# ErlerPhilipp/points2surf

Hardware: NVIDIA H100
Metric: SDF queries/sec at grid_res=256 (higher is better)
Workload: dtype f16 operands / f32 accumulate (wgmma); hi/lo split f16 (fp32-level) for FC tails and guard-band recompute

## Files before the change

points2surf_b200/csrc/net_tc.cu:

```cuda
#include "model.cuh"
#include "tc_ptx.cuh"

namespace p2s {

using namespace ptx;

namespace {

constexpr int kTile = 64;
constexpr int kWG = 2;
constexpr int kThreads = 128 * kWG;
constexpr uint32_t kAct2Bytes = kTile * 128 * 2;
template <bool PRECISE>
struct Cfg {
    static constexpr int kChunks = PRECISE ? 1 : 4;
    static constexpr int kSplit = 8 / kChunks;
    static constexpr uint32_t kChunkBytes = PRECISE ? 65536u : 32768u;
    static constexpr uint32_t kW3Bytes = kChunks * kChunkBytes;
    static constexpr uint32_t kMidScale = PRECISE ? 2u : 1u;
    static constexpr uint32_t kMidBytes = (8192u + 8192u + 16384u) * kMidScale;
    static constexpr uint32_t kPerqBytes = PRECISE ? 16384u : 8192u;
    static constexpr uint32_t kOffMid = kW3Bytes;
    static constexpr uint32_t kWgPerq = kAct2Bytes * kMidScale;
    static constexpr uint32_t kWgWq = kWgPerq + kPerqBytes;
    static constexpr uint32_t kWgBytes = kWgWq + 192 * 4;
    static constexpr uint32_t kOffWg = kOffMid + kMidBytes;
    static constexpr uint32_t kOffBias = kOffWg + kWG * kWgBytes;
    static constexpr uint32_t kSmemBytes = kOffBias + 320 * 4;
};
static_assert(Cfg<false>::kSmemBytes <= 232448 && Cfg<true>::kSmemBytes <= 232448, "shared memory budget");

struct Seg {
    const float* ptr;
    int n;
    int tiles;
    int center;
};

struct PassParams {
    Seg seg[2];
    const float* query;
    const float* R;
    int tiles_per_query;
    int B;
    const float* W0;
    const float* b0;
    int num_mid;
    int mid_N[3];
    const uint8_t* mid_img[3];
    const float* mid_bias[3];
    int perq_layer;
    const uint8_t* perq_img;
    const uint8_t* w3_img;
    float* out;
};

__device__ __forceinline__ uint32_t pack_relu(float a, float b) {
    uint32_t r;
    asm("cvt.rn.relu.satfinite.f16x2.f32 %0, %1, %2;" : "=r"(r) : "f"(b), "f"(a));
    return r;
}
__device__ __forceinline__ void pack_relu_split(float a, float b, uint32_t& hi, uint32_t& lo) {
    hi = pack_relu(a, b);
    const float2 hf = __half22float2(*reinterpret_cast<const __half2*>(&hi));
    lo = pack_half2(fmaxf(a, 0.f) - hf.x, fmaxf(b, 0.f) - hf.y);
}
template <bool PRECISE>
__device__ __forceinline__ void pack_act(float a, float b, uint32_t& hi, uint32_t& lo) {
    if (PRECISE) pack_relu_split(a, b, hi, lo);
    else hi = pack_relu(a, b);
}

template <bool PRECISE, int R>
__device__ __forceinline__ void mid_mma(float (&d)[R], const uint32_t (&a)[4], const uint32_t (&al)[4], uint64_t w, uint64_t w_lo, uint32_t acc) {
    if (R == 32) {
        auto& d32 = reinterpret_cast<float (&)[32]>(d);
        if (PRECISE) { wgmma_rs_n64(d32, al, w, acc); wgmma_rs_n64(d32, a, w_lo, 1); wgmma_rs_n64(d32, a, w, 1); }
        else wgmma_rs_n64(d32, a, w, acc);
    } else {
        auto& d64 = reinterpret_cast<float (&)[64]>(d);
        if (PRECISE) { wgmma_rs_n128(d64, al, w, acc); wgmma_rs_n128(d64, a, w_lo, 1); wgmma_rs_n128(d64, a, w, 1); }
        else wgmma_rs_n128(d64, a, w, acc);
    }
}

template <bool PRECISE>
__global__ void __launch_bounds__(kThreads, 1) pointnet_pass_kernel(const PassParams p) {
    using C = Cfg<PRECISE>;
    constexpr int kL = PRECISE ? 4 : 1;
    extern __shared__ __align__(1024) uint8_t smem[];
    float* s_bias = reinterpret_cast<float*>(smem + C::kOffBias);
    const int tid = threadIdx.x, wg = tid >> 7, t = tid & 127, lane = tid & 31, q4 = lane & 3;
    const int r0 = (t >> 5) * 16 + (lane >> 2);
    const int part = blockIdx.x % C::kSplit;
    const int stream = blockIdx.x / C::kSplit, nstreams = gridDim.x / C::kSplit;
    const int nq = (p.B > stream) ? (p.B - stream + nstreams - 1) / nstreams : 0;
    const int tpq = p.tiles_per_query;
    uint32_t mid_off[3] = {0, 0, 0};
    {
        uint32_t o = 0;
        for (int l = 0; l < p.num_mid; ++l) { mid_off[l] = o; o += (uint32_t)p.mid_N[l] * 128u * C::kMidScale; }
    }

    if (nq > 0) {
        const uint4* src = reinterpret_cast<const uint4*>(p.w3_img + (size_t)part * C::kW3Bytes);
        uint4* dst = reinterpret_cast<uint4*>(smem);
        for (uint32_t i = tid; i < C::kW3Bytes / 16; i += kThreads) dst[i] = src[i];
        for (int l = 0; l < p.num_mid; ++l) {
            if (l == p.perq_layer) continue;
            const uint4* s = reinterpret_cast<const uint4*>(p.mid_img[l]);
            uint4* d = reinterpret_cast<uint4*>(smem + C::kOffMid + mid_off[l]);
            for (uint32_t i = tid; i < (uint32_t)p.mid_N[l] * 8u * C::kMidScale; i += kThreads) d[i] = s[i];
        }
    }
    {
        int off = 0;
        for (int l = 0; l < p.num_mid; ++l) {
            for (int i = tid; i < p.mid_N[l]; i += kThreads) s_bias[off + i] = p.mid_bias[l][i];
            off += p.mid_N[l];
        }
        for (int i = tid; i < 64; i += kThreads) s_bias[256 + i] = p.b0[i];
    }
    fence_proxy_async_smem();
    __syncthreads();

    uint8_t* wsm = smem + C::kOffWg + wg * C::kWgBytes;
    uint8_t* act2 = wsm;
    uint8_t* perq = wsm + C::kWgPerq;
    float* wq = reinterpret_cast<float*>(wsm + C::kWgWq);
    const float* s_b0 = s_bias + 256;
    const uint32_t bar_id = 1 + (uint32_t)wg;
    auto wg_sync = [&]() { asm volatile("bar.sync %0, 128;" ::"r"(bar_id) : "memory"); };
    const uint64_t dsc_act2 = make_smem_desc(smem_u32(act2), 128, 2048);
    const uint64_t dsc_w3 = make_smem_desc(smem_u32(smem), 128, 2048);
    uint64_t dsc_mid[3], dsc_mid_lo[3];
    for (int l = 0; l < 3; ++l) {
        const bool pq = l == p.perq_layer;
        dsc_mid[l] = make_smem_desc(pq ? smem_u32(perq) : smem_u32(smem + C::kOffMid) + mid_off[l], 128, 1024);
        dsc_mid_lo[l] = dsc_mid[l] + (uint64_t)((pq ? 8192u : (uint32_t)p.mid_N[l] * 128u) >> 4);
    }

    for (int qi = wg; qi < nq; qi += kWG) {
        const size_t q = (size_t)stream + (size_t)qi * nstreams;
        wg_sync();
        if (t < 64) {
            const float w0 = p.W0[t * 3 + 0], w1 = p.W0[t * 3 + 1], w2 = p.W0[t * 3 + 2];
            float r[9] = {1.f, 0.f, 0.f, 0.f, 1.f, 0.f, 0.f, 0.f, 1.f};
            if (p.R) {
#pragma unroll
                for (int i = 0; i < 9; ++i) r[i] = p.R[q * 9 + i];
            }
            wq[0 * 64 + t] = w0 * r[0] + w1 * r[3] + w2 * r[6];
            wq[1 * 64 + t] = w0 * r[1] + w1 * r[4] + w2 * r[7];
            wq[2 * 64 + t] = w0 * r[2] + w1 * r[5] + w2 * r[8];
        }
        if (p.perq_layer >= 0) {
            const uint4* s = reinterpret_cast<const uint4*>(p.perq_img + q * C::kPerqBytes);
            uint4* d = reinterpret_cast<uint4*>(perq);
            for (uint32_t i = t; i < C::kPerqBytes / 16; i += 128) d[i] = s[i];
            fence_proxy_async_smem();
        }
        wg_sync();
        float rmax[4 * C::kChunks];
#pragma unroll
        for (int i = 0; i < 4 * C::kChunks; ++i) rmax[i] = -INFINITY;
        for (int tq = 0; tq < tpq; ++tq) {
            const int sgi = tq < p.seg[0].tiles ? 0 : 1;
            const Seg& sg = p.seg[sgi];
            float cx = 0.f, cy = 0.f, cz = 0.f;
            if (sg.center) { cx = p.query[q * 3 + 0]; cy = p.query[q * 3 + 1]; cz = p.query[q * 3 + 2]; }
            float px[2], py[2], pz[2];
#pragma unroll
            for (int h = 0; h < 2; ++h) {
                int local = (tq - (sgi ? p.seg[0].tiles : 0)) * kTile + r0 + 8 * h;
                if (local >= sg.n) local = 0;
                const float* src = sg.ptr + (q * sg.n + local) * 3;
                px[h] = src[0] - cx; py[h] = src[1] - cy; pz[h] = src[2] - cz;
            }
            uint32_t a[4][4], al[4][kL];
#pragma unroll
            for (int kk = 0; kk < 4; ++kk) {
#pragma unroll
                for (int hc = 0; hc < 2; ++hc) {
                    const int ch = kk * 16 + hc * 8 + 2 * q4;
                    const float2 wx = *reinterpret_cast<const float2*>(wq + 0 * 64 + ch);
                    const float2 wy = *reinterpret_cast<const float2*>(wq + 1 * 64 + ch);
                    const float2 wz = *reinterpret_cast<const float2*>(wq + 2 * 64 + ch);
                    const float2 bb = *reinterpret_cast<const float2*>(s_b0 + ch);
#pragma unroll
                    for (int h = 0; h < 2; ++h) {
                        const float v0 = fmaf(wx.x, px[h], fmaf(wy.x, py[h], fmaf(wz.x, pz[h], bb.x)));
                        const float v1 = fmaf(wx.y, px[h], fmaf(wy.y, py[h], fmaf(wz.y, pz[h], bb.y)));
                        pack_act<PRECISE>(v0, v1, a[kk][hc * 2 + h], al[kk][PRECISE ? hc * 2 + h : 0]);
                    }
                }
            }
            int boff = 0;
            for (int l = 0; l < p.num_mid; ++l) {
                const float* bl = s_bias + boff;
                const uint64_t w = dsc_mid[l], w_lo = dsc_mid_lo[l];
                if (l < p.num_mid - 1) {
                    float d[32];
#pragma unroll
                    for (int i = 0; i < 32; ++i) d[i] = 0.f;
                    wgmma_fence();
#pragma unroll
                    for (int ks = 0; ks < 4; ++ks)
                        mid_mma<PRECISE>(d, a[ks], reinterpret_cast<const uint32_t (&)[4]>(al[PRECISE ? ks : 0]), w + (uint64_t)(ks * 16), w_lo + (uint64_t)(ks * 16), ks > 0);
                    wgmma_commit();
                    wgmma_wait<0>();
                    fence_regs(d);
#pragma unroll
                    for (int j = 0; j < 8; ++j) {
                        const float2 bb = *reinterpret_cast<const float2*>(bl + 8 * j + 2 * q4);
                        pack_act<PRECISE>(d[4 * j] + bb.x, d[4 * j + 1] + bb.y, a[j >> 1][(j & 1) * 2], al[j >> 1][PRECISE ? (j & 1) * 2 : 0]);
                        pack_act<PRECISE>(d[4 * j + 2] + bb.x, d[4 * j + 3] + bb.y, a[j >> 1][(j & 1) * 2 + 1], al[j >> 1][PRECISE ? (j & 1) * 2 + 1 : 0]);
                    }
                } else {
                    float d[64];
#pragma unroll
                    for (int i = 0; i < 64; ++i) d[i] = 0.f;
                    wgmma_fence();
#pragma unroll
                    for (int ks = 0; ks < 4; ++ks)
                        mid_mma<PRECISE>(d, a[ks], reinterpret_cast<const uint32_t (&)[4]>(al[PRECISE ? ks : 0]), w + (uint64_t)(ks * 16), w_lo + (uint64_t)(ks * 16), ks > 0);
                    wgmma_commit();
                    wgmma_wait<0>();
                    fence_regs(d);
                    wg_sync();
#pragma unroll
                    for (int j = 0; j < 16; ++j) {
                        const int k = 8 * j + 2 * q4;
                        const float2 bb = *reinterpret_cast<const float2*>(bl + k);
#pragma unroll
                        for (int h = 0; h < 2; ++h) {
                            const int pt = r0 + 8 * h;
                            const uint32_t off = (uint32_t)(pt >> 3) * 2048u + (uint32_t)j * 128u + (uint32_t)(pt & 7) * 16u + (uint32_t)q4 * 4u;
                            uint32_t hi, lo = 0;
                            pack_act<PRECISE>(d[4 * j + 2 * h] + bb.x, d[4 * j + 2 * h + 1] + bb.y, hi, lo);
                            *reinterpret_cast<uint32_t*>(act2 + off) = hi;
                            if (PRECISE) *reinterpret_cast<uint32_t*>(act2 + kAct2Bytes + off) = lo;
                        }
                    }
                    fence_proxy_async_smem();
                    wg_sync();
                }
                boff += p.mid_N[l];
            }
#pragma unroll
            for (int c = 0; c < C::kChunks; ++c) {
                float d0[32], d1[32];
#pragma unroll
                for (int i = 0; i < 32; ++i) { d0[i] = 0.f; d1[i] = 0.f; }
                const uint64_t wa = dsc_w3 + (uint64_t)((uint32_t)c * (C::kChunkBytes >> 4)), wb = wa + (uint64_t)(16384u >> 4);
                wgmma_fence();
#pragma unroll
                for (int ks = 0; ks < 8; ++ks) {
                    const uint64_t x = dsc_act2 + (uint64_t)(ks * 16), o = (uint64_t)(ks * 16);
                    if (PRECISE) {
                        const uint64_t x_lo = x + (uint64_t)(kAct2Bytes >> 4), lo = (uint64_t)(32768u >> 4);
                        wgmma_ss_n64(d0, wa + lo + o, x, ks > 0); wgmma_ss_n64(d0, wa + o, x_lo, 1); wgmma_ss_n64(d0, wa + o, x, 1);
                        wgmma_ss_n64(d1, wb + lo + o, x, ks > 0); wgmma_ss_n64(d1, wb + o, x_lo, 1); wgmma_ss_n64(d1, wb + o, x, 1);
                    } else {
                        wgmma_ss_n64(d0, wa + o, x, ks > 0);
                        wgmma_ss_n64(d1, wb + o, x, ks > 0);
                    }
                }
                wgmma_commit();
                wgmma_wait<0>();
                fence_regs(d0);
                fence_regs(d1);
#pragma unroll
                for (int j = 0; j < 8; ++j) {
                    rmax[4 * c + 0] = fmaxf(rmax[4 * c + 0], fmaxf(d0[4 * j], d0[4 * j + 1]));
                    rmax[4 * c + 1] = fmaxf(rmax[4 * c + 1], fmaxf(d0[4 * j + 2], d0[4 * j + 3]));
                    rmax[4 * c + 2] = fmaxf(rmax[4 * c + 2], fmaxf(d1[4 * j], d1[4 * j + 1]));
                    rmax[4 * c + 3] = fmaxf(rmax[4 * c + 3], fmaxf(d1[4 * j + 2], d1[4 * j + 3]));
                }
            }
        }
#pragma unroll
        for (int i = 0; i < 4 * C::kChunks; ++i) {
            rmax[i] = fmaxf(rmax[i], __shfl_xor_sync(0xffffffffu, rmax[i], 1));
            rmax[i] = fmaxf(rmax[i], __shfl_xor_sync(0xffffffffu, rmax[i], 2));
        }
        if (q4 == 0) {
#pragma unroll
            for (int i = 0; i < 4 * C::kChunks; ++i)
                p.out[q * 1024 + (size_t)((part * C::kChunks + (i >> 2)) * 128 + ((i >> 1) & 1) * 64 + r0 + (i & 1) * 8)] = rmax[i];
        }
    }
}

__global__ void pack_kmajor_kernel(const float* __restrict__ W, int rows, int K, int row0, uint32_t sbo, uint8_t* __restrict__ img, int lo) {
    int e = blockIdx.x * blockDim.x + threadIdx.x;
    if (e >= rows * K) return;
    int r = e / K, k = e % K;
    uint32_t off = (uint32_t)(r >> 3) * sbo + (uint32_t)(k >> 3) * 128u + (uint32_t)(r & 7) * 16u + (uint32_t)(k & 7) * 2u;
    const float w = W[(size_t)(row0 + r) * K + k];
    const __half h = __float2half_rn(w);
    *reinterpret_cast<__half*>(img + off) = lo ? __float2half_rn(w - __half2float(h)) : h;
}

__global__ void pack_perq_kernel(const float* __restrict__ W, int64_t B, uint8_t* __restrict__ img) {
    int64_t e = (int64_t)blockIdx.x * blockDim.x + threadIdx.x;
    if (e >= B * 4096) return;
    int64_t b = e >> 12;
    int r = (int)((e >> 6) & 63), k = (int)(e & 63);
    uint32_t off = (uint32_t)(r >> 3) * 1024u + (uint32_t)(k >> 3) * 128u + (uint32_t)(r & 7) * 16u + (uint32_t)(k & 7) * 2u;
    *reinterpret_cast<__half*>(img + b * 8192 + off) = __float2half_rn(W[e]);
}

__global__ void __launch_bounds__(256) fold_w1_kernel(const float* __restrict__ W1, const float* __restrict__ T, int64_t B, uint8_t* __restrict__ img) {
    __shared__ float sW[64][65];
    __shared__ __align__(16) float sT[64][68];
    const int64_t b = blockIdx.x;
    const int tid = threadIdx.x;
    for (int e = tid; e < 4096; e += 256) {
        const int r = e >> 6, c = e & 63;
        sW[r][c] = W1[e];
        sT[r][c] = T[b * 4096 + e] + (r == c ? 1.0f : 0.0f);
    }
    __syncthreads();
    const int o = tid >> 2, i0 = (tid & 3) * 16;
    float acc[16];
#pragma unroll
    for (int i = 0; i < 16; ++i) acc[i] = 0.f;
    for (int j = 0; j < 64; ++j) {
        const float w = sW[o][j];
#pragma unroll
        for (int i4 = 0; i4 < 4; ++i4) {
            const float4 t4 = *reinterpret_cast<const float4*>(&sT[j][i0 + 4 * i4]);
            acc[4 * i4 + 0] = fmaf(w, t4.x, acc[4 * i4 + 0]);
            acc[4 * i4 + 1] = fmaf(w, t4.y, acc[4 * i4 + 1]);
            acc[4 * i4 + 2] = fmaf(w, t4.z, acc[4 * i4 + 2]);
            acc[4 * i4 + 3] = fmaf(w, t4.w, acc[4 * i4 + 3]);
        }
    }
    uint8_t* dst = img + b * 8192 + (uint32_t)(o >> 3) * 1024u + (uint32_t)(o & 7) * 16u;
#pragma unroll
    for (int h = 0; h < 2; ++h) {
        uint32_t v[4];
#pragma unroll
        for (int e = 0; e < 4; ++e) v[e] = pack_half2(acc[h * 8 + 2 * e], acc[h * 8 + 2 * e + 1]);
        *reinterpret_cast<uint4*>(dst + (uint32_t)(i0 / 8 + h) * 128u) = make_uint4(v[0], v[1], v[2], v[3]);
    }
}

__global__ void fold_fc3_kernel(const float* __restrict__ W1, const float* __restrict__ Wfc3, const float* __restrict__ bfc3,
                                float* __restrict__ G, float* __restrict__ g0) {
    const int oi = blockIdx.x;
    const int o = oi >> 6, i = oi & 63;
    const int k = threadIdx.x;
    float acc = 0.f;
    for (int j = 0; j < 64; ++j) acc = fmaf(W1[o * 64 + j], Wfc3[(size_t)(j * 64 + i) * 256 + k], acc);
    G[(size_t)oi * 256 + k] = acc;
    if (k == 0) {
        float b = W1[o * 64 + i];
        for (int j = 0; j < 64; ++j) b = fmaf(W1[o * 64 + j], bfc3[j * 64 + i], b);
        g0[oi] = b;
    }
}

__global__ void transpose64_kernel(const float* __restrict__ in, float* __restrict__ out, int64_t B) {
    int64_t e = (int64_t)blockIdx.x * blockDim.x + threadIdx.x;
    if (e >= B * 4096) return;
    int64_t b = e >> 12;
    int i = (int)((e >> 6) & 63), j = (int)(e & 63);
    out[e] = in[b * 4096 + j * 64 + i];
}

__global__ void guard_flag_kernel(const float* __restrict__ logits, int64_t B, float band, int32_t* __restrict__ list, int* __restrict__ count, int64_t base, int64_t cap) {
    int64_t i = (int64_t)blockIdx.x * blockDim.x + threadIdx.x;
    if (i >= B) return;
    if (fabsf(logits[i * 2 + 1]) < band) {
        int slot = atomicAdd(count, 1);
        if (slot < cap) list[slot] = (int32_t)(base + i);
    }
}
__global__ void guard_gather_kernel(const float* __restrict__ src, const int32_t* __restrict__ list, int n, int row_floats, float* __restrict__ dst) {
    int64_t e = (int64_t)blockIdx.x * blockDim.x + threadIdx.x;
    if (e >= (int64_t)n * row_floats) return;
    int i = (int)(e / row_floats), j = (int)(e % row_floats);
    dst[e] = src[(int64_t)list[i] * row_floats + j];
}
__global__ void guard_scatter_kernel(const float* __restrict__ src, const int32_t* __restrict__ list, int n, float* __restrict__ logits) {
    int i = blockIdx.x * blockDim.x + threadIdx.x;
    if (i >= n) return;
    logits[(int64_t)list[i] * 2 + 0] = src[i * 2 + 0];
    logits[(int64_t)list[i] * 2 + 1] = src[i * 2 + 1];
}
__global__ void guard_scatter_rows_kernel(const float* __restrict__ src, const int32_t* __restrict__ list, int n, int row_floats, float* __restrict__ dst) {
    int64_t e = (int64_t)blockIdx.x * blockDim.x + threadIdx.x;
    if (e >= (int64_t)n * row_floats) return;
    int i = (int)(e / row_floats), j = (int)(e % row_floats);
    dst[(int64_t)list[i] * row_floats + j] = src[e];
}

}

struct TcStack {
    uint8_t* w3_img = nullptr;
    uint8_t* mid_img[3] = {nullptr, nullptr, nullptr};
    uint8_t* w3_img_p = nullptr;
    uint8_t* mid_img_p[3] = {nullptr, nullptr, nullptr};
    const float* mid_bias[3] = {nullptr, nullptr, nullptr};
    int mid_N[3] = {0, 0, 0};
    int num_mid = 0;
    const float* W0 = nullptr;
    const float* b0 = nullptr;
    const float* b3 = nullptr;
};

struct TcFc {
    const Layer* L = nullptr;
    const uint8_t* img = nullptr;
};
struct TcStnFc { TcFc fc1, fc2, fc3; };

struct TcWeights {
    TcStack qstn;
    TcStack stn[2], fin[2];
    TcStnFc qstn_fc, stn_fc[2];
    TcFc head_fc1[2], head_fc2, head_fc3;
    const uint8_t* fold_img[2] = {nullptr, nullptr};
    const float* fold_bias[2] = {nullptr, nullptr};
    bool fc_on_tc = true;
    std::vector<void*> allocs;
    int sm_count = 132;
    bool prof_on = false;
    std::vector<std::pair<cudaEvent_t, cudaEvent_t>> prof_events;
    double prof_flops = 0.0;
    ~TcWeights() {
        for (void* a : allocs) cudaFree(a);
        for (auto& e : prof_events) { cudaEventDestroy(e.first); cudaEventDestroy(e.second); }
    }
};

namespace {

uint8_t* tc_alloc(TcWeights& t, size_t bytes) {
    void* p = nullptr;
    P2S_CUDA(cudaMalloc(&p, bytes));
    P2S_CUDA(cudaMemset(p, 0, bytes));
    t.allocs.push_back(p);
    return (uint8_t*)p;
}

uint8_t* pack_layer(TcWeights& t, const Layer& L, uint32_t sbo, bool split = false) {
    const size_t one = (size_t)L.cout * L.cin * 2;
    uint8_t* img = tc_alloc(t, one * (split ? 2 : 1));
    P2S_LAUNCH(pack_kmajor_kernel, (unsigned)cdiv((int64_t)L.cout * L.cin, 256), 256, 0, 0, L.W, L.cout, L.cin, 0, sbo, img, 0);
    if (split) P2S_LAUNCH(pack_kmajor_kernel, (unsigned)cdiv((int64_t)L.cout * L.cin, 256), 256, 0, 0, L.W, L.cout, L.cin, 0, sbo, img + one, 1);
    return img;
}

uint8_t* pack_w3(TcWeights& t, const Layer& L, bool split = false) {
    P2S_CHECK(L.cout == 1024 && L.cin == 128, "big layer must be 128 -> 1024");
    const size_t chunk = split ? 65536 : 32768;
    uint8_t* img = tc_alloc(t, 8 * chunk);
    for (int c = 0; c < 8; ++c) {
        P2S_LAUNCH(pack_kmajor_kernel, (unsigned)cdiv(128 * 128, 256), 256, 0, 0, L.W, 128, 128, c * 128, 2048u, img + (size_t)c * chunk, 0);
        if (split) P2S_LAUNCH(pack_kmajor_kernel, (unsigned)cdiv(128 * 128, 256), 256, 0, 0, L.W, 128, 128, c * 128, 2048u, img + (size_t)c * chunk + 32768, 1);
    }
    return img;
}

void launch_pass(Model& m, const TcStack& s, const Seg& s0, const Seg& s1, const float* query, const float* R,
                 int64_t B, int perq_layer, const uint8_t* perq_img, float* out, cudaStream_t st, bool precise) {
    PassParams p{};
    p.seg[0] = s0; p.seg[1] = s1;
    p.query = query; p.R = R;
    p.tiles_per_query = s0.tiles + s1.tiles;
    p.B = (int)B;
    p.W0 = s.W0; p.b0 = s.b0;
    p.num_mid = s.num_mid;
    for (int l = 0; l < 3; ++l) { p.mid_N[l] = s.mid_N[l]; p.mid_img[l] = precise ? s.mid_img_p[l] : s.mid_img[l]; p.mid_bias[l] = s.mid_bias[l]; }
    p.perq_layer = perq_layer;
    p.perq_img = perq_img;
    p.w3_img = precise ? s.w3_img_p : s.w3_img;
    p.out = out;
    for (int l = 0; l < s.num_mid; ++l)
        P2S_CHECK(s.mid_N[l] == (l == s.num_mid - 1 ? 128 : 64), "pass kernel: mid layers must be 64 -> 64 ... -> 128");
    TcWeights& t = *m.tc;
    const int split = precise ? Cfg<true>::kSplit : Cfg<false>::kSplit;
    int streams = t.sm_count / split;
    if ((int64_t)streams > B) streams = (int)B;
    const int grid = streams * split;
    cudaEvent_t e0 = nullptr, e1 = nullptr;
    const bool prof = t.prof_on && !precise;
    if (prof) {
        P2S_CUDA(cudaEventCreate(&e0)); P2S_CUDA(cudaEventCreate(&e1));
        P2S_CUDA(cudaEventRecord(e0, st));
    }
    if (precise) P2S_LAUNCH(pointnet_pass_kernel<true>, grid, kThreads, Cfg<true>::kSmemBytes, st, p);
    else P2S_LAUNCH(pointnet_pass_kernel<false>, grid, kThreads, Cfg<false>::kSmemBytes, st, p);
    if (prof) {
        P2S_CUDA(cudaEventRecord(e1, st));
        t.prof_events.emplace_back(e0, e1);
        double mac_pt = 3.0 * 64 + 128.0 * 1024;
        int prev = 64;
        for (int l = 0; l < s.num_mid; ++l) { mac_pt += (double)prev * s.mid_N[l]; prev = s.mid_N[l]; }
        t.prof_flops += 2.0 * mac_pt * (double)(s0.n + s1.n) * (double)B;
    }
}

Seg make_seg(const float* ptr, int n, int center) { return Seg{ptr, n, n > 0 ? (n + kTile - 1) / kTile : 0, center}; }

void run_fc(const TcFc& f, const float* in, int lda, float* out, int ldc, int64_t Bc, bool relu, bool on_tc, cudaStream_t st,
            const float* in_bias = nullptr, bool in_relu = false) {
    const Layer& L = *f.L;
    if (on_tc && f.img) launch_fc_tc(in, lda, f.img, L.b, out, ldc, Bc, L.cout, L.cin, relu, st, 0, in_bias, in_relu);
    else {
        P2S_CHECK(!in_bias, "input bias needs the tensor-core FC kernel");
        launch_gemm_nt(in, 0, lda, L.W, 0, L.b, out, 0, ldc, (int)Bc, L.cout, L.cin, 1, relu, st);
    }
}

void fc_tail(const Layer& b3src, const TcStnFc& s, bool on_tc, const float* gmax_raw, int64_t Bc, float* g, float* f1, float* f2, float* out, cudaStream_t st) {
    if (on_tc && s.fc1.img) run_fc(s.fc1, gmax_raw, 1024, f1, 512, Bc, true, true, st, b3src.b, true);
    else {
        P2S_CUDA(cudaMemcpyAsync(g, gmax_raw, (size_t)Bc * 1024 * 4, cudaMemcpyDeviceToDevice, st));
        launch_bias_act(g, b3src.b, Bc, 1024, true, st);
        run_fc(s.fc1, g, 1024, f1, 512, Bc, true, on_tc, st);
    }
    run_fc(s.fc2, f1, 512, f2, 256, Bc, true, on_tc, st);
    run_fc(s.fc3, f2, 256, out, s.fc3.L->cout, Bc, false, on_tc, st);
}

}

void tc_build(Model& m) {
    P2S_CHECK(m.cfg.net_size == 1024, "tensor-core path needs net_size 1024");
    TcWeights* t = new TcWeights();
    m.tc = t;
    cudaDeviceProp prop;
    P2S_CUDA(cudaGetDeviceProperties(&prop, m.device));
    t->sm_count = prop.multiProcessorCount;
    P2S_CUDA(cudaFuncSetAttribute(pointnet_pass_kernel<false>, cudaFuncAttributeMaxDynamicSharedMemorySize, (int)Cfg<false>::kSmemBytes));
    P2S_CUDA(cudaFuncSetAttribute(pointnet_pass_kernel<true>, cudaFuncAttributeMaxDynamicSharedMemorySize, (int)Cfg<true>::kSmemBytes));
    auto build_stn = [&](TcStack& s, const Stn& stn, const Layer* c0a, const Layer* c0b) {
        if (!c0a) {
            s.W0 = stn.c1.W; s.b0 = stn.c1.b;
            s.num_mid = 1;
            s.mid_img[0] = pack_layer(*t, stn.c2, 1024); s.mid_bias[0] = stn.c2.b; s.mid_N[0] = 128;
            s.mid_img_p[0] = pack_layer(*t, stn.c2, 1024, true);
        } else {
            s.W0 = c0a->W; s.b0 = c0a->b;
            s.num_mid = 3;
            s.mid_img[0] = pack_layer(*t, *c0b, 1024); s.mid_bias[0] = c0b->b; s.mid_N[0] = 64;
            s.mid_img[1] = pack_layer(*t, stn.c1, 1024); s.mid_bias[1] = stn.c1.b; s.mid_N[1] = 64;
            s.mid_img[2] = pack_layer(*t, stn.c2, 1024); s.mid_bias[2] = stn.c2.b; s.mid_N[2] = 128;
            s.mid_img_p[0] = pack_layer(*t, *c0b, 1024, true);
            s.mid_img_p[1] = pack_layer(*t, stn.c1, 1024, true);
            s.mid_img_p[2] = pack_layer(*t, stn.c2, 1024, true);
        }
        s.w3_img_p = pack_w3(*t, stn.c3, true);
        s.w3_img = pack_w3(*t, stn.c3);
        s.b3 = stn.c3.b;
    };
    auto build_fin = [&](TcStack& s, const Feat& f) {
        s.W0 = f.conv0a.W; s.b0 = f.conv0a.b;
        s.num_mid = 3;
        s.mid_img[0] = pack_layer(*t, f.conv0b, 1024); s.mid_bias[0] = f.conv0b.b; s.mid_N[0] = 64;
        s.mid_img[1] = nullptr; s.mid_bias[1] = f.conv1.b; s.mid_N[1] = 64;
        s.mid_img[2] = pack_layer(*t, f.conv2, 1024); s.mid_bias[2] = f.conv2.b; s.mid_N[2] = 128;
        s.mid_img_p[0] = pack_layer(*t, f.conv0b, 1024, true);
        s.mid_img_p[2] = pack_layer(*t, f.conv2, 1024, true);
        s.w3_img_p = pack_w3(*t, f.conv3, true);
        s.w3_img = pack_w3(*t, f.conv3);
        s.b3 = f.conv3.b;
    };
    fc_tc_init();
    t->fc_on_tc = !env_flag("P2S_FC_FP32");
    auto mk_fc = [&](const Layer& L) {
        TcFc f;
        f.L = &L;
        f.img = fc_tc_supported(L.cout, L.cin) ? fc_tc_pack(L, t->allocs) : nullptr;
        return f;
    };
    auto mk_stn_fc = [&](const Stn& s) { TcStnFc r; r.fc1 = mk_fc(s.fc1); r.fc2 = mk_fc(s.fc2); r.fc3 = mk_fc(s.fc3); return r; };
    if (m.shared_qstn) t->qstn_fc = mk_stn_fc(m.point_stn);
    else if (m.global.has_qstn) t->qstn_fc = mk_stn_fc(m.global.stn1);
    t->stn_fc[0] = mk_stn_fc(m.local.stn2);
    t->stn_fc[1] = mk_stn_fc(m.global.stn2);
    for (int br = 0; br < 2; ++br) {
        const Feat& f = br ? m.global : m.local;
        P2S_CHECK(f.stn2.fc3.cout == 4096 && f.stn2.fc3.cin == 256 && f.conv1.cout == 64 && f.conv1.cin == 64, "unexpected STN shape");
        float* G = reinterpret_cast<float*>(tc_alloc(*t, (size_t)4096 * 256 * 4));
        float* g0 = reinterpret_cast<float*>(tc_alloc(*t, 4096 * 4));
        P2S_LAUNCH(fold_fc3_kernel, 4096, 256, 0, 0, f.conv1.W, f.stn2.fc3.W, f.stn2.fc3.b, G, g0);
        t->fold_img[br] = fc_tc_pack_raw(G, 4096, 256, t->allocs);
// ... 186 lines not shown
```

points2surf_b200/csrc/tc_ptx.cuh:

```cuda
#pragma once
#include <cstdint>
#include <cuda_fp16.h>

namespace p2s {
namespace ptx {

__device__ __forceinline__ uint32_t smem_u32(const void* p) { return (uint32_t)__cvta_generic_to_shared(p); }

__device__ __forceinline__ void mbar_init(uint64_t* bar, uint32_t count) {
    asm volatile("mbarrier.init.shared::cta.b64 [%0], %1;" ::"r"(smem_u32(bar)), "r"(count) : "memory");
}
__device__ __forceinline__ void fence_mbar_init() { asm volatile("fence.mbarrier_init.release.cluster;" ::: "memory"); }
__device__ __forceinline__ void mbar_arrive(uint64_t* bar) {
    asm volatile("mbarrier.arrive.shared::cta.b64 _, [%0];" ::"r"(smem_u32(bar)) : "memory");
}
__device__ __forceinline__ void mbar_arrive_expect_tx(uint64_t* bar, uint32_t bytes) {
    asm volatile("mbarrier.arrive.expect_tx.shared::cta.b64 _, [%0], %1;" ::"r"(smem_u32(bar)), "r"(bytes) : "memory");
}
__device__ __forceinline__ bool mbar_try_wait(uint64_t* bar, uint32_t parity) {
    uint32_t ok;
    asm volatile(
        "{\n\t.reg .pred p;\n\t"
        "mbarrier.try_wait.parity.shared::cta.b64 p, [%1], %2;\n\t"
        "selp.u32 %0, 1, 0, p;\n\t}"
        : "=r"(ok) : "r"(smem_u32(bar)), "r"(parity) : "memory");
    return ok != 0;
}
__device__ __forceinline__ void mbar_wait_bounded(uint64_t* bar, uint32_t parity) {
    long long t0 = clock64();
    while (!mbar_try_wait(bar, parity)) {
        if (clock64() - t0 > 2000000000LL) __trap();
    }
}
__device__ __forceinline__ bool mbar_test_wait(uint64_t* bar, uint32_t parity) {
    uint32_t ok;
    asm volatile(
        "{\n\t.reg .pred p;\n\t"
        "mbarrier.test_wait.parity.shared::cta.b64 p, [%1], %2;\n\t"
        "selp.u32 %0, 1, 0, p;\n\t}"
        : "=r"(ok) : "r"(smem_u32(bar)), "r"(parity) : "memory");
    return ok != 0;
}
__device__ __forceinline__ void mbar_wait(uint64_t* bar, uint32_t parity) {
    while (!mbar_try_wait(bar, parity)) {}
}

__device__ __forceinline__ bool elect_one() {
    uint32_t pred;
    asm volatile("{\n\t.reg .pred P1;\n\telect.sync _|P1, 0xffffffff;\n\tselp.u32 %0, 1, 0, P1;\n\t}" : "=r"(pred));
    return pred != 0;
}

__device__ __forceinline__ void fence_proxy_async_smem() { asm volatile("fence.proxy.async.shared::cta;" ::: "memory"); }

__device__ __forceinline__ void bulk_g2s(void* smem_dst, const void* gmem_src, uint32_t bytes, uint64_t* bar) {
    asm volatile("cp.async.bulk.shared::cluster.global.mbarrier::complete_tx::bytes [%0], [%1], %2, [%3];"
                 ::"r"(smem_u32(smem_dst)), "l"(gmem_src), "r"(bytes), "r"(smem_u32(bar)) : "memory");
}

__device__ __forceinline__ uint64_t make_smem_desc(uint32_t smem_addr, uint32_t lbo_bytes, uint32_t sbo_bytes) {
    uint64_t d = 0;
    d |= (uint64_t)((smem_addr & 0x3FFFFu) >> 4);
    d |= (uint64_t)((lbo_bytes >> 4) & 0x3FFFu) << 16;
    d |= (uint64_t)((sbo_bytes >> 4) & 0x3FFFu) << 32;
    return d;
}

__device__ __forceinline__ void wgmma_fence() { asm volatile("wgmma.fence.sync.aligned;" ::: "memory"); }
__device__ __forceinline__ void wgmma_commit() { asm volatile("wgmma.commit_group.sync.aligned;" ::: "memory"); }
template <int N>
__device__ __forceinline__ void wgmma_wait() { asm volatile("wgmma.wait_group.sync.aligned %0;" ::"n"(N) : "memory"); }
template <int R>
__device__ __forceinline__ void fence_regs(float (&d)[R]) {
#pragma unroll
    for (int i = 0; i < R; ++i) asm volatile("" : "+f"(d[i])::"memory");
}
__device__ __forceinline__ void wgmma_rs_n64(float (&d)[32], const uint32_t (&a)[4], uint64_t b_desc, uint32_t accumulate) {
    asm volatile(
        "{\n\t.reg .pred p;\n\tsetp.ne.b32 p, %37, 0;\n\t"
        "wgmma.mma_async.sync.aligned.m64n64k16.f32.f16.f16 {%0, %1, %2, %3, %4, %5, %6, %7, %8, %9, %10, %11, %12, %13, %14, %15, %16, %17, %18, %19, %20, %21, %22, %23, %24, %25, %26, %27, %28, %29, %30, %31}, {%32, %33, %34, %35}, %36, p, 1, 1, 0;\n\t}"
        : "+f"(d[0]), "+f"(d[1]), "+f"(d[2]), "+f"(d[3]), "+f"(d[4]), "+f"(d[5]), "+f"(d[6]), "+f"(d[7]), "+f"(d[8]), "+f"(d[9]), "+f"(d[10]), "+f"(d[11]), "+f"(d[12]), "+f"(d[13]), "+f"(d[14]), "+f"(d[15]), "+f"(d[16]), "+f"(d[17]), "+f"(d[18]), "+f"(d[19]), "+f"(d[20]), "+f"(d[21]), "+f"(d[22]), "+f"(d[23]), "+f"(d[24]), "+f"(d[25]), "+f"(d[26]), "+f"(d[27]), "+f"(d[28]), "+f"(d[29]), "+f"(d[30]), "+f"(d[31])
        : "r"(a[0]), "r"(a[1]), "r"(a[2]), "r"(a[3]), "l"(b_desc), "r"(accumulate) : "memory");
}
__device__ __forceinline__ void wgmma_rs_n128(float (&d)[64], const uint32_t (&a)[4], uint64_t b_desc, uint32_t accumulate) {
    asm volatile(
        "{\n\t.reg .pred p;\n\tsetp.ne.b32 p, %69, 0;\n\t"
        "wgmma.mma_async.sync.aligned.m64n128k16.f32.f16.f16 {%0, %1, %2, %3, %4, %5, %6, %7, %8, %9, %10, %11, %12, %13, %14, %15, %16, %17, %18, %19, %20, %21, %22, %23, %24, %25, %26, %27, %28, %29, %30, %31, %32, %33, %34, %35, %36, %37, %38, %39, %40, %41, %42, %43, %44, %45, %46, %47, %48, %49, %50, %51, %52, %53, %54, %55, %56, %57, %58, %59, %60, %61, %62, %63}, {%64, %65, %66, %67}, %68, p, 1, 1, 0;\n\t}"
        : "+f"(d[0]), "+f"(d[1]), "+f"(d[2]), "+f"(d[3]), "+f"(d[4]), "+f"(d[5]), "+f"(d[6]), "+f"(d[7]), "+f"(d[8]), "+f"(d[9]), "+f"(d[10]), "+f"(d[11]), "+f"(d[12]), "+f"(d[13]), "+f"(d[14]), "+f"(d[15]), "+f"(d[16]), "+f"(d[17]), "+f"(d[18]), "+f"(d[19]), "+f"(d[20]), "+f"(d[21]), "+f"(d[22]), "+f"(d[23]), "+f"(d[24]), "+f"(d[25]), "+f"(d[26]), "+f"(d[27]), "+f"(d[28]), "+f"(d[29]), "+f"(d[30]), "+f"(d[31]), "+f"(d[32]), "+f"(d[33]), "+f"(d[34]), "+f"(d[35]), "+f"(d[36]), "+f"(d[37]), "+f"(d[38]), "+f"(d[39]), "+f"(d[40]), "+f"(d[41]), "+f"(d[42]), "+f"(d[43]), "+f"(d[44]), "+f"(d[45]), "+f"(d[46]), "+f"(d[47]), "+f"(d[48]), "+f"(d[49]), "+f"(d[50]), "+f"(d[51]), "+f"(d[52]), "+f"(d[53]), "+f"(d[54]), "+f"(d[55]), "+f"(d[56]), "+f"(d[57]), "+f"(d[58]), "+f"(d[59]), "+f"(d[60]), "+f"(d[61]), "+f"(d[62]), "+f"(d[63])
        : "r"(a[0]), "r"(a[1]), "r"(a[2]), "r"(a[3]), "l"(b_desc), "r"(accumulate) : "memory");
}
__device__ __forceinline__ void wgmma_ss_n64(float (&d)[32], uint64_t a_desc, uint64_t b_desc, uint32_t accumulate) {
    asm volatile(
        "{\n\t.reg .pred p;\n\tsetp.ne.b32 p, %34, 0;\n\t"
        "wgmma.mma_async.sync.aligned.m64n64k16.f32.f16.f16 {%0, %1, %2, %3, %4, %5, %6, %7, %8, %9, %10, %11, %12, %13, %14, %15, %16, %17, %18, %19, %20, %21, %22, %23, %24, %25, %26, %27, %28, %29, %30, %31}, %32, %33, p, 1, 1, 0, 0;\n\t}"
        : "+f"(d[0]), "+f"(d[1]), "+f"(d[2]), "+f"(d[3]), "+f"(d[4]), "+f"(d[5]), "+f"(d[6]), "+f"(d[7]), "+f"(d[8]), "+f"(d[9]), "+f"(d[10]), "+f"(d[11]), "+f"(d[12]), "+f"(d[13]), "+f"(d[14]), "+f"(d[15]), "+f"(d[16]), "+f"(d[17]), "+f"(d[18]), "+f"(d[19]), "+f"(d[20]), "+f"(d[21]), "+f"(d[22]), "+f"(d[23]), "+f"(d[24]), "+f"(d[25]), "+f"(d[26]), "+f"(d[27]), "+f"(d[28]), "+f"(d[29]), "+f"(d[30]), "+f"(d[31])
        : "l"(a_desc), "l"(b_desc), "r"(accumulate) : "memory");
}
__device__ __forceinline__ void wgmma_ss_n128(float (&d)[64], uint64_t a_desc, uint64_t b_desc, uint32_t accumulate) {
    asm volatile(
        "{\n\t.reg .pred p;\n\tsetp.ne.b32 p, %66, 0;\n\t"
        "wgmma.mma_async.sync.aligned.m64n128k16.f32.f16.f16 {%0, %1, %2, %3, %4, %5, %6, %7, %8, %9, %10, %11, %12, %13, %14, %15, %16, %17, %18, %19, %20, %21, %22, %23, %24, %25, %26, %27, %28, %29, %30, %31, %32, %33, %34, %35, %36, %37, %38, %39, %40, %41, %42, %43, %44, %45, %46, %47, %48, %49, %50, %51, %52, %53, %54, %55, %56, %57, %58, %59, %60, %61, %62, %63}, %64, %65, p, 1, 1, 0, 0;\n\t}"
        : "+f"(d[0]), "+f"(d[1]), "+f"(d[2]), "+f"(d[3]), "+f"(d[4]), "+f"(d[5]), "+f"(d[6]), "+f"(d[7]), "+f"(d[8]), "+f"(d[9]), "+f"(d[10]), "+f"(d[11]), "+f"(d[12]), "+f"(d[13]), "+f"(d[14]), "+f"(d[15]), "+f"(d[16]), "+f"(d[17]), "+f"(d[18]), "+f"(d[19]), "+f"(d[20]), "+f"(d[21]), "+f"(d[22]), "+f"(d[23]), "+f"(d[24]), "+f"(d[25]), "+f"(d[26]), "+f"(d[27]), "+f"(d[28]), "+f"(d[29]), "+f"(d[30]), "+f"(d[31]), "+f"(d[32]), "+f"(d[33]), "+f"(d[34]), "+f"(d[35]), "+f"(d[36]), "+f"(d[37]), "+f"(d[38]), "+f"(d[39]), "+f"(d[40]), "+f"(d[41]), "+f"(d[42]), "+f"(d[43]), "+f"(d[44]), "+f"(d[45]), "+f"(d[46]), "+f"(d[47]), "+f"(d[48]), "+f"(d[49]), "+f"(d[50]), "+f"(d[51]), "+f"(d[52]), "+f"(d[53]), "+f"(d[54]), "+f"(d[55]), "+f"(d[56]), "+f"(d[57]), "+f"(d[58]), "+f"(d[59]), "+f"(d[60]), "+f"(d[61]), "+f"(d[62]), "+f"(d[63])
        : "l"(a_desc), "l"(b_desc), "r"(accumulate) : "memory");
}

__device__ __forceinline__ uint32_t pack_half2(float lo, float hi) {
    __half2 h = __floats2half2_rn(lo, hi);
    return *reinterpret_cast<uint32_t*>(&h);
}

}
}
```

Before: 401,000.

## Keep last-layer activations in registers and swap operand roles for final GEMM

The final mid-layer output is no longer staged to shared memory. It is packed directly into register A-fragments, and the big feature GEMM now uses register-sourced wgmma with the activations as A and the W3 chunk as B (n128). This removes the smem write, proxy fence and two workgroup barriers per tile. Because the output layout becomes points-by-channels, the max-pool is redone with an in-warp shuffle halving tree plus a cross-warp smem reduction at the end of each query. The cost is much higher register pressure, since a3/al3 hold 8x4 fragments (more in precise mode) alongside the 64-float accumulator.

```diff
diff --git a/points2surf_b200/csrc/net_tc.cu b/points2surf_b200/csrc/net_tc.cu
--- a/points2surf_b200/csrc/net_tc.cu
+++ b/points2surf_b200/csrc/net_tc.cu
@@ -10,7 +10,6 @@
 constexpr int kTile = 64;
 constexpr int kWG = 2;
 constexpr int kThreads = 128 * kWG;
-constexpr uint32_t kAct2Bytes = kTile * 128 * 2;
 template <bool PRECISE>
 struct Cfg {
     static constexpr int kChunks = PRECISE ? 1 : 4;
@@ -21,7 +20,7 @@
     static constexpr uint32_t kMidBytes = (8192u + 8192u + 16384u) * kMidScale;
     static constexpr uint32_t kPerqBytes = PRECISE ? 16384u : 8192u;
     static constexpr uint32_t kOffMid = kW3Bytes;
-    static constexpr uint32_t kWgPerq = kAct2Bytes * kMidScale;
+    static constexpr uint32_t kWgPerq = 4u * kChunks * 128u * 4u;
     static constexpr uint32_t kWgWq = kWgPerq + kPerqBytes;
     static constexpr uint32_t kWgBytes = kWgWq + 192 * 4;
     static constexpr uint32_t kOffWg = kOffMid + kMidBytes;
@@ -84,6 +83,26 @@
     }
 }
 
+template <bool PRECISE, int S, int L>
+__device__ __forceinline__ void acc_to_a(const float (&d)[8 * S], const float* bias, int q4, uint32_t (&a)[S][4], uint32_t (&al)[S][L]) {
+#pragma unroll
+    for (int j = 0; j < 2 * S; ++j) {
+        const float2 bb = *reinterpret_cast<const float2*>(bias + 8 * j + 2 * q4);
+        pack_act<PRECISE>(d[4 * j] + bb.x, d[4 * j + 1] + bb.y, a[j >> 1][(j & 1) * 2], al[j >> 1][PRECISE ? (j & 1) * 2 : 0]);
+        pack_act<PRECISE>(d[4 * j + 2] + bb.x, d[4 * j + 3] + bb.y, a[j >> 1][(j & 1) * 2 + 1], al[j >> 1][PRECISE ? (j & 1) * 2 + 1 : 0]);
+    }
+}
+
+template <int H>
+__device__ __forceinline__ void max_halve(float (&m)[32], int lane, int x) {
+    const bool up = (lane & x) != 0;
+#pragma unroll
+    for (int i = 0; i < H; ++i) {
+        const float keep = up ? m[i + H] : m[i], give = up ? m[i] : m[i + H];
+        m[i] = fmaxf(keep, __shfl_xor_sync(0xffffffffu, give, x));
+    }
+}
+
 template <bool PRECISE>
 __global__ void __launch_bounds__(kThreads, 1) pointnet_pass_kernel(const PassParams p) {
     using C = Cfg<PRECISE>;
@@ -125,13 +144,12 @@
     __syncthreads();
 
     uint8_t* wsm = smem + C::kOffWg + wg * C::kWgBytes;
-    uint8_t* act2 = wsm;
+    float* red = reinterpret_cast<float*>(wsm);
     uint8_t* perq = wsm + C::kWgPerq;
     float* wq = reinterpret_cast<float*>(wsm + C::kWgWq);
     const float* s_b0 = s_bias + 256;
     const uint32_t bar_id = 1 + (uint32_t)wg;
     auto wg_sync = [&]() { asm volatile("bar.sync %0, 128;" ::"r"(bar_id) : "memory"); };
-    const uint64_t dsc_act2 = make_smem_desc(smem_u32(act2), 128, 2048);
     const uint64_t dsc_w3 = make_smem_desc(smem_u32(smem), 128, 2048);
     uint64_t dsc_mid[3], dsc_mid_lo[3];
     for (int l = 0; l < 3; ++l) {
@@ -195,6 +213,7 @@
                     }
                 }
             }
+            uint32_t a3[8][4], al3[8][kL];
             int boff = 0;
             for (int l = 0; l < p.num_mid; ++l) {
                 const float* bl = s_bias + boff;
@@ -210,12 +229,7 @@
                     wgmma_commit();
                     wgmma_wait<0>();
                     fence_regs(d);
-#pragma unroll
-                    for (int j = 0; j < 8; ++j) {
-                        const float2 bb = *reinterpret_cast<const float2*>(bl + 8 * j + 2 * q4);
-                        pack_act<PRECISE>(d[4 * j] + bb.x, d[4 * j + 1] + bb.y, a[j >> 1][(j & 1) * 2], al[j >> 1][PRECISE ? (j & 1) * 2 : 0]);
-                        pack_act<PRECISE>(d[4 * j + 2] + bb.x, d[4 * j + 3] + bb.y, a[j >> 1][(j & 1) * 2 + 1], al[j >> 1][PRECISE ? (j & 1) * 2 + 1 : 0]);
-                    }
+                    acc_to_a<PRECISE>(d, bl, q4, a, al);
                 } else {
                     float d[64];
 #pragma unroll
@@ -227,67 +241,60 @@
                     wgmma_commit();
                     wgmma_wait<0>();
                     fence_regs(d);
-                    wg_sync();
-#pragma unroll
-                    for (int j = 0; j < 16; ++j) {
-                        const int k = 8 * j + 2 * q4;
-                        const float2 bb = *reinterpret_cast<const float2*>(bl + k);
-#pragma unroll
-                        for (int h = 0; h < 2; ++h) {
-                            const int pt = r0 + 8 * h;
-                            const uint32_t off = (uint32_t)(pt >> 3) * 2048u + (uint32_t)j * 128u + (uint32_t)(pt & 7) * 16u + (uint32_t)q4 * 4u;
-                            uint32_t hi, lo = 0;
-                            pack_act<PRECISE>(d[4 * j + 2 * h] + bb.x, d[4 * j + 2 * h + 1] + bb.y, hi, lo);
-                            *reinterpret_cast<uint32_t*>(act2 + off) = hi;
-                            if (PRECISE) *reinterpret_cast<uint32_t*>(act2 + kAct2Bytes + off) = lo;
-                        }
-                    }
-                    fence_proxy_async_smem();
-                    wg_sync();
+                    acc_to_a<PRECISE>(d, bl, q4, a3, al3);
                 }
                 boff += p.mid_N[l];
             }
 #pragma unroll
             for (int c = 0; c < C::kChunks; ++c) {
-                float d0[32], d1[32];
-#pragma unroll
-                for (int i = 0; i < 32; ++i) { d0[i] = 0.f; d1[i] = 0.f; }
-                const uint64_t wa = dsc_w3 + (uint64_t)((uint32_t)c * (C::kChunkBytes >> 4)), wb = wa + (uint64_t)(16384u >> 4);
+                float d[64];
+#pragma unroll
+                for (int i = 0; i < 64; ++i) d[i] = 0.f;
+                const uint64_t w = dsc_w3 + (uint64_t)((uint32_t)c * (C::kChunkBytes >> 4));
                 wgmma_fence();
 #pragma unroll
                 for (int ks = 0; ks < 8; ++ks) {
-                    const uint64_t x = dsc_act2 + (uint64_t)(ks * 16), o = (uint64_t)(ks * 16);
+                    const uint64_t o = (uint64_t)(ks * 16);
                     if (PRECISE) {
-                        const uint64_t x_lo = x + (uint64_t)(kAct2Bytes >> 4), lo = (uint64_t)(32768u >> 4);
-                        wgmma_ss_n64(d0, wa + lo + o, x, ks > 0); wgmma_ss_n64(d0, wa + o, x_lo, 1); wgmma_ss_n64(d0, wa + o, x, 1);
-                        wgmma_ss_n64(d1, wb + lo + o, x, ks > 0); wgmma_ss_n64(d1, wb + o, x_lo, 1); wgmma_ss_n64(d1, wb + o, x, 1);
+                        const uint64_t lo = (uint64_t)(32768u >> 4);
+                        wgmma_rs_n128(d, a3[ks], w + lo + o, ks > 0);
+                        wgmma_rs_n128(d, reinterpret_cast<const uint32_t (&)[4]>(al3[PRECISE ? ks : 0]), w + o, 1);
+                        wgmma_rs_n128(d, a3[ks], w + o, 1);
                     } else {
-                        wgmma_ss_n64(d0, wa + o, x, ks > 0);
-                        wgmma_ss_n64(d1, wb + o, x, ks > 0);
+                        wgmma_rs_n128(d, a3[ks], w + o, ks > 0);
                     }
                 }
                 wgmma_commit();
                 wgmma_wait<0>();
-                fence_regs(d0);
-                fence_regs(d1);
-#pragma unroll
-                for (int j = 0; j < 8; ++j) {
-                    rmax[4 * c + 0] = fmaxf(rmax[4 * c + 0], fmaxf(d0[4 * j], d0[4 * j + 1]));
-                    rmax[4 * c + 1] = fmaxf(rmax[4 * c + 1], fmaxf(d0[4 * j + 2], d0[4 * j + 3]));
-                    rmax[4 * c + 2] = fmaxf(rmax[4 * c + 2], fmaxf(d1[4 * j], d1[4 * j + 1]));
-                    rmax[4 * c + 3] = fmaxf(rmax[4 * c + 3], fmaxf(d1[4 * j + 2], d1[4 * j + 3]));
+                fence_regs(d);
+                float m[32];
+#pragma unroll
+                for (int j = 0; j < 16; ++j) {
+                    m[2 * j] = fmaxf(d[4 * j], d[4 * j + 2]);
+                    m[2 * j + 1] = fmaxf(d[4 * j + 1], d[4 * j + 3]);
                 }
+                max_halve<16>(m, lane, 16);
+                max_halve<8>(m, lane, 8);
+                max_halve<4>(m, lane, 4);
+#pragma unroll
+                for (int i = 0; i < 4; ++i) rmax[4 * c + i] = fmaxf(rmax[4 * c + i], m[i]);
             }
         }
-#pragma unroll
-        for (int i = 0; i < 4 * C::kChunks; ++i) {
-            rmax[i] = fmaxf(rmax[i], __shfl_xor_sync(0xffffffffu, rmax[i], 1));
-            rmax[i] = fmaxf(rmax[i], __shfl_xor_sync(0xffffffffu, rmax[i], 2));
-        }
-        if (q4 == 0) {
-#pragma unroll
-            for (int i = 0; i < 4 * C::kChunks; ++i)
-                p.out[q * 1024 + (size_t)((part * C::kChunks + (i >> 2)) * 128 + ((i >> 1) & 1) * 64 + r0 + (i & 1) * 8)] = rmax[i];
+        const int warp = t >> 5, cb = 16 * (lane >> 2) + 2 * q4;
+#pragma unroll
+        for (int c = 0; c < C::kChunks; ++c) {
+            float* r = red + warp * (C::kChunks * 128) + c * 128 + cb;
+            *reinterpret_cast<float2*>(r) = make_float2(rmax[4 * c + 0], rmax[4 * c + 1]);
+            *reinterpret_cast<float2*>(r + 8) = make_float2(rmax[4 * c + 2], rmax[4 * c + 3]);
+        }
+        wg_sync();
+#pragma unroll
+        for (int c = 0; c < C::kChunks; ++c) {
+            const int ch = c * 128 + t;
+            float v = red[ch];
+#pragma unroll
+            for (int w = 1; w < 4; ++w) v = fmaxf(v, red[w * (C::kChunks * 128) + ch]);
+            p.out[q * 1024 + (size_t)(part * C::kChunks * 128 + ch)] = v;
         }
     }
 }
diff --git a/points2surf_b200/csrc/tc_ptx.cuh b/points2surf_b200/csrc/tc_ptx.cuh
--- a/points2surf_b200/csrc/tc_ptx.cuh
+++ b/points2surf_b200/csrc/tc_ptx.cuh
@@ -89,13 +89,6 @@
         : "+f"(d[0]), "+f"(d[1]), "+f"(d[2]), "+f"(d[3]), "+f"(d[4]), "+f"(d[5]), "+f"(d[6]), "+f"(d[7]), "+f"(d[8]), "+f"(d[9]), "+f"(d[10]), "+f"(d[11]), "+f"(d[12]), "+f"(d[13]), "+f"(d[14]), "+f"(d[15]), "+f"(d[16]), "+f"(d[17]), "+f"(d[18]), "+f"(d[19]), "+f"(d[20]), "+f"(d[21]), "+f"(d[22]), "+f"(d[23]), "+f"(d[24]), "+f"(d[25]), "+f"(d[26]), "+f"(d[27]), "+f"(d[28]), "+f"(d[29]), "+f"(d[30]), "+f"(d[31]), "+f"(d[32]), "+f"(d[33]), "+f"(d[34]), "+f"(d[35]), "+f"(d[36]), "+f"(d[37]), "+f"(d[38]), "+f"(d[39]), "+f"(d[40]), "+f"(d[41]), "+f"(d[42]), "+f"(d[43]), "+f"(d[44]), "+f"(d[45]), "+f"(d[46]), "+f"(d[47]), "+f"(d[48]), "+f"(d[49]), "+f"(d[50]), "+f"(d[51]), "+f"(d[52]), "+f"(d[53]), "+f"(d[54]), "+f"(d[55]), "+f"(d[56]), "+f"(d[57]), "+f"(d[58]), "+f"(d[59]), "+f"(d[60]), "+f"(d[61]), "+f"(d[62]), "+f"(d[63])
         : "r"(a[0]), "r"(a[1]), "r"(a[2]), "r"(a[3]), "l"(b_desc), "r"(accumulate) : "memory");
 }
-__device__ __forceinline__ void wgmma_ss_n64(float (&d)[32], uint64_t a_desc, uint64_t b_desc, uint32_t accumulate) {
-    asm volatile(
-        "{\n\t.reg .pred p;\n\tsetp.ne.b32 p, %34, 0;\n\t"
-        "wgmma.mma_async.sync.aligned.m64n64k16.f32.f16.f16 {%0, %1, %2, %3, %4, %5, %6, %7, %8, %9, %10, %11, %12, %13, %14, %15, %16, %17, %18, %19, %20, %21, %22, %23, %24, %25, %26, %27, %28, %29, %30, %31}, %32, %33, p, 1, 1, 0, 0;\n\t}"
-        : "+f"(d[0]), "+f"(d[1]), "+f"(d[2]), "+f"(d[3]), "+f"(d[4]), "+f"(d[5]), "+f"(d[6]), "+f"(d[7]), "+f"(d[8]), "+f"(d[9]), "+f"(d[10]), "+f"(d[11]), "+f"(d[12]), "+f"(d[13]), "+f"(d[14]), "+f"(d[15]), "+f"(d[16]), "+f"(d[17]), "+f"(d[18]), "+f"(d[19]), "+f"(d[20]), "+f"(d[21]), "+f"(d[22]), "+f"(d[23]), "+f"(d[24]), "+f"(d[25]), "+f"(d[26]), "+f"(d[27]), "+f"(d[28]), "+f"(d[29]), "+f"(d[30]), "+f"(d[31])
-        : "l"(a_desc), "l"(b_desc), "r"(accumulate) : "memory");
-}
 __device__ __forceinline__ void wgmma_ss_n128(float (&d)[64], uint64_t a_desc, uint64_t b_desc, uint32_t accumulate) {
     asm volatile(
         "{\n\t.reg .pred p;\n\tsetp.ne.b32 p, %66, 0;\n\t"
```

Result: faster. 407,300, median of 6 (+1.6%).
